# SKA-INAF/caesar-mrcnn

Hardware: AMD Instinct MI355X
Metric: train images/sec (whole node) + detect ms/image, ResNet-101 256x256 (higher is better)
Workload: dtype f32; 1 GPU; resnet101+FPN 256x256 3-class (+bg), nimg_per_gpu=4, train step (fwd+bwd+SGD), 512 train ROIs, 2000 proposals; global_batch=4, parallelism=dp1, weights=random init (Keras defaults)

## Files before the change

caesar-mrcnn_amd/_hip.py:

```python
import ctypes as C
import os
import threading

PKG_DIR = os.path.dirname(os.path.abspath(__file__))
LIB_PATH = os.path.join(PKG_DIR, "libmrcnn_hip.so")


class HipPathError(RuntimeError):
    pass


class ConvDesc(C.Structure):
    _fields_ = [(n, C.c_int32) for n in (
        "N", "H", "W", "Cin", "Cout", "KH", "KW", "stride", "pad_t", "pad_l", "OH", "OW",
        "act", "res_mode", "out_mode", "cmod")] + [
        ("out_n_stride", C.c_int64), ("out_h_stride", C.c_int64), ("out_w_stride", C.c_int64)]


class ConvProblem(C.Structure):
    _fields_ = [("d", ConvDesc)] + [(n, C.c_void_p) for n in ("x", "w", "bias", "scale", "shift", "res", "out", "z_out")]


class WgradProblem(C.Structure):
    _fields_ = [("d", ConvDesc), ("x", C.c_void_p), ("dy", C.c_void_p), ("dw", C.c_void_p), ("accumulate", C.c_int32)]
# ... 125 lines not shown
    "mrcnn_conv2d_wgrad_h16": (C.c_int, [C.POINTER(ConvDesc), C.c_int, _P, _P, _P, _P, C.c_size_t, C.c_int, C.c_float, _P]),
    "mrcnn_mask_out_fwd_h16": (C.c_int, [C.c_int, _P, _P, _P, _P, C.c_int64, C.c_int, C.c_int, _P]),
    "mrcnn_mask_out_bwd_h16": (C.c_int, [C.c_int] + [_P] * 8 + [C.c_int64, C.c_int, C.c_int, C.c_int, C.c_int, C.c_float, _P]),
    "mrcnn_weights_to_h16": (C.c_int, [_P, _P, _P, C.c_int, C.c_int, C.c_int, C.c_int, C.c_int, _P]),
    "mrcnn_weights_to_h16_batched": (C.c_int, [_P, _P, C.c_int, C.c_int, C.c_int, _P]),
    "mrcnn_cast_to_h16": (C.c_int, [_P, _P, C.c_int64, C.c_int, C.c_float, _P]),
    "mrcnn_epilogue_bwd_h16": (C.c_int, [C.c_int] + [_P] * 10 + [C.c_int64, C.c_int, C.c_int, C.c_float, _P]),
    "mrcnn_epilogue_bwd_h16_dy": (C.c_int, [C.c_int] + [_P] * 11 + [C.c_int64, C.c_int, C.c_int, C.c_float, _P]),
    "mrcnn_cast_from_h16": (C.c_int, [_P, _P, C.c_int64, C.c_int, C.c_float, _P]),
    "mrcnn_axpy_from_h16": (C.c_int, [_P, _P, C.c_int64, C.c_int, C.c_float, _P]),
    "mrcnn_rpn_targets_workspace": (C.c_size_t, [C.POINTER(RpnTargetDesc)]),
    "mrcnn_rpn_targets": (C.c_int, [C.POINTER(RpnTargetDesc)] + [_P] * 7 + [C.c_size_t, _P]),
    "mrcnn_detection_workspace": (C.c_size_t, [C.POINTER(DetectionDesc)]),
    "mrcnn_detection_fwd": (C.c_int, [C.POINTER(DetectionDesc)] + [_P] * 6 + [C.c_size_t, _P]),
    "mrcnn_losses_workspace": (C.c_size_t, [C.POINTER(LossDesc)]),
    "mrcnn_losses_fwd_bwd": (C.c_int, [C.POINTER(LossDesc)] + [_P] * 18 + [C.c_size_t, _P]),
    "mrcnn_grad_prepare": (C.c_int, [_P, _P, C.c_float, _P, C.c_int64, _P, _P]),
    "mrcnn_sumsq": (C.c_int, [_P, C.c_int64, _P, _P]),
    "mrcnn_sgd_momentum": (C.c_int, [_P, _P, _P, _P, C.c_float, C.c_float, C.c_float, _P, C.c_int64, _P]),
    "mrcnn_sgd_momentum_guarded": (C.c_int, [_P, _P, _P, _P, C.c_float, C.c_float, C.c_float, _P, C.c_int64, _P, _P]),
    "mrcnn_winograd_buffer_floats": (C.c_size_t, [C.c_int, C.c_int, C.c_int, C.c_int, C.c_int]),
    "mrcnn_winograd_weights": (C.c_int, [_P, _P, C.c_int, C.c_int, C.c_int, _P]),
    "mrcnn_gemm_batched_f32": (C.c_int, [_P, _P, _P, C.c_int, C.c_int, C.c_int, C.c_int, _P]),
    "mrcnn_winograd_gemm": (C.c_int, [_P, _P, _P, C.c_int, C.c_int, C.c_int, C.c_int, _P]),
    "mrcnn_winograd_group_floats": (C.c_size_t, [C.POINTER(WinoGroup), C.c_int, C.c_int]),
    "mrcnn_winograd_input_g": (C.c_int, [_P, _P, C.c_int, C.c_int, C.c_int, C.c_int, C.POINTER(WinoGroup), _P]),
    "mrcnn_winograd_weights_g": (C.c_int, [_P, _P, C.c_int, C.c_int, C.c_int, C.c_int, _P]),
    "mrcnn_winograd_output_g": (C.c_int, [_P, _P, _P, _P, _P, _P, C.c_int, C.c_int, C.c_int, C.c_int, C.c_int, C.POINTER(WinoGroup), _P]),
    "mrcnn_winograd_output_bwd_g": (C.c_int, [_P, _P, _P, _P, _P, _P, _P, _P, _P, _P, C.c_int, C.c_int, C.c_int, C.c_int, C.c_int,
                                             C.POINTER(WinoGroup), _P]),
    "mrcnn_winograd_output_bwd_zmask_g": (C.c_int, [_P] * 10 + [C.c_int, C.c_int, C.c_int, C.c_int, C.POINTER(WinoGroup), _P]),
    "mrcnn_winograd_dy_g": (C.c_int, [_P, _P, C.c_int, C.c_int, C.c_int, C.c_int, C.POINTER(WinoGroup), _P]),
    "mrcnn_winograd_dw_g": (C.c_int, [_P, _P, C.c_int, C.c_int, C.c_int, C.c_int, C.c_int, _P]),
    "mrcnn_deconv2x2_gemm": (C.c_int, [_P, _P, _P, _P, C.c_int, C.c_int, C.c_int, C.c_int, C.c_int, C.c_int, _P]),
    "mrcnn_allreduce_load": (C.c_int, [C.c_char_p]),
    "mrcnn_allreduce_unique_id": (C.c_int, [_P]),
    "mrcnn_allreduce_init": (C.c_int, [C.POINTER(_P), _P, C.c_int, C.c_int]),
    "mrcnn_allreduce_scratch": (C.c_size_t, [C.c_int, C.c_int64, C.c_int]),
    "mrcnn_allreduce_grad": (C.c_int, [_P, _P, C.c_int64, C.c_int64, C.c_int, _P, C.c_size_t, _P]),
    "mrcnn_allreduce_direct_plan": (C.c_int, [C.c_int, C.c_int, C.c_int64, C.c_int64, C.c_int, _P, _P, _P, _P]),
    "mrcnn_allreduce_direct_simulate": (C.c_int, [_P, _P, C.c_size_t, C.c_int, C.c_int64, C.c_int64, _P]),
    "mrcnn_allreduce_destroy": (C.c_int, [_P]),
    "mrcnn_allreduce_last_error": (C.c_char_p, []),
    "mrcnn_tuning_set": (C.c_int, [C.c_char_p, C.c_longlong]),
    "mrcnn_hip_version": (C.c_char_p, []),
}

_lib = None
_proxy = None
_tape = None
_tape_owner = None

_NO_RECORD = ("_workspace", "_tiles_check", "_outline_check", "_draw_check", "_supported", "_status_offset", "_version", "mrcnn_allreduce_", "_scratch", "_floats")


class _LibProxy(object):

    def __init__(self, real):
        self._real = real

    def __getattr__(self, name):
        real = getattr(self._real, name)
        if any(k in name for k in _NO_RECORD):
            f = real
        else:
            def f(*args, _real=real):
# ... 103 lines not shown
```

caesar-mrcnn_amd/csrc/conv_wgrad.hip:

```cpp
#include "common.h"
#include <type_traits>
#include <cstdlib>

struct WgradArgs {
    const float* x; const float* dy; float* out;
    int N, H, W, Cin, Cout, KH, KW, stride, pad_t, pad_l, OH, OW;
    int M, Ktot, fast, splits, chunk, acc;
    FastDiv d_ohw, d_ow;
    const PixelEntry* table;
};

template <int BI, int BN, int WM, int WN>
__global__ __launch_bounds__(WM * WN * 64, 2) void conv_wgrad_kernel(const WgradArgs p) {
    constexpr int NT = WM * WN * 64;
    constexpr int TM = BI / WM / 32, TN = BN / WN / 32;
    constexpr int XST = BI + 4, YST = BN + 4;
    constexpr int XV = 8 * BI / NT, YV = 8 * BN / NT;
    __shared__ __attribute__((aligned(16))) float lds[32 * XST + 32 * YST];
    float* Xs = lds;
    float* Ys = lds + 32 * XST;

    const int tid = threadIdx.x, lane = tid & 63, wave = tid >> 6;
    const int wm = wave / WN, wn = wave % WN;
    const int ntiles = (p.Cout + BN - 1) / BN;
    const int itiles = (p.Ktot + BI - 1) / BI;
    int bid = blockIdx.x;
    const int ntile = bid % ntiles; bid /= ntiles;
    const int itile = bid % itiles;
    const int split = bid / itiles;
    const int i0 = itile * BI, n0 = ntile * BN;
    const int m_begin = split * p.chunk;
    const int m_end = (m_begin + p.chunk < p.M) ? m_begin + p.chunk : p.M;
    const int tap = i0 / p.Cin, ci0 = i0 - tap * p.Cin;
    const int kh = tap / p.KW, kw = tap - kh * p.KW;
    const int ohw = p.OH * p.OW;
// ... 598 lines not shown
    long long blocks = 0, rblocks = 0;
    for (int g = 0; g < n; ++g) {
        const mrcnn_wgrad_problem& q = problems[g];
        const mrcnn_conv_desc* d = &q.d;
        if (!q.x || !q.dy || !q.dw) return MRCNN_ERR_ARG;
        if ((reinterpret_cast<uintptr_t>(q.x) | reinterpret_cast<uintptr_t>(q.dy) | reinterpret_cast<uintptr_t>(q.dw)) & 15)
            return MRCNN_ERR_UNSUPPORTED;
        const long long M = (long long)d->N * d->OH * d->OW;
        WgradArgs& a = mp.a[g];
        a.x = q.x; a.dy = q.dy;
        a.out = pl.splits[g] > 1 ? (float*)((char*)workspace + pl.slab_off[g]) : q.dw;
        a.N = d->N; a.H = d->H; a.W = d->W; a.Cin = d->Cin; a.Cout = d->Cout; a.KH = d->KH; a.KW = d->KW;
        a.stride = d->stride; a.pad_t = d->pad_t; a.pad_l = d->pad_l; a.OH = d->OH; a.OW = d->OW;
        a.M = (int)M; a.Ktot = d->KH * d->KW * d->Cin; a.fast = 1; a.splits = pl.splits[g]; a.chunk = pl.chunk[g];
        a.acc = q.accumulate;
        a.d_ohw = make_fastdiv((unsigned)(d->OH * d->OW)); a.d_ow = make_fastdiv((unsigned)d->OW);
        a.table = nullptr;
        const long long xbytes = (long long)d->N * d->H * d->W * d->Cin * 4;
        const long long shift = ((long long)d->pad_t * d->W + d->pad_l) * d->Cin * 4;
        mp.x_shift[g] = (unsigned)shift; mp.x_records[g] = (unsigned)(xbytes + shift);
        mp.dw[g] = q.dw;
        mp.first[g] = (int)blocks;
        blocks += (long long)(a.Ktot / 128) * (a.Cout / 128) * a.splits;
        mp.rfirst[g] = (int)rblocks;
        if (a.splits > 1) rblocks += cdiv64((long long)a.Ktot * a.Cout / 4, 256);
    }
    for (int g = n; g <= WGRAD_MULTI_MAX; ++g) { mp.first[g] = (int)blocks; mp.rfirst[g] = (int)rblocks; }
    hipStream_t s = (hipStream_t)stream;
    hipLaunchKernelGGL((conv_wgrad_blds_multi_kernel<WGRAD_BP>), dim3((unsigned)blocks), dim3(256), 0, s, mp);
    if (rblocks > 0) hipLaunchKernelGGL(wgrad_reduce_multi_kernel, dim3((unsigned)rblocks), dim3(256), 0, s, mp);
    return mrcnn_launch_status();
}

__global__ void flip_transpose_kernel(const float* __restrict__ w, float* wt, int KH, int KW, int Cin, int Cout) {
    __shared__ float tile[32][33];
    const int tap = blockIdx.z;
    const int kh = tap / KW, kw = tap % KW;
    const int tap_t = (KH - 1 - kh) * KW + (KW - 1 - kw);
    const int ci0 = blockIdx.y * 32, co0 = blockIdx.x * 32;
    const int tx = threadIdx.x & 31, ty = threadIdx.x >> 5;
    for (int r = ty; r < 32; r += 8) {
        int ci = ci0 + r, co = co0 + tx;
        tile[r][tx] = (ci < Cin && co < Cout) ? w[((long long)tap * Cin + ci) * Cout + co] : 0.f;
    }
    __syncthreads();
    for (int r = ty; r < 32; r += 8) {
        int co = co0 + r, ci = ci0 + tx;
        if (co < Cout && ci < Cin) wt[((long long)tap_t * Cout + co) * Cin + ci] = tile[tx][r];
    }
}

extern "C" int mrcnn_weight_flip_transpose(const float* w, float* w_t, int KH, int KW, int Cin, int Cout, void* stream) {
    if (!w || !w_t || KH <= 0 || KW <= 0 || Cin <= 0 || Cout <= 0) return MRCNN_ERR_ARG;
    dim3 grid((Cout + 31) / 32, (Cin + 31) / 32, KH * KW);
    hipLaunchKernelGGL(flip_transpose_kernel, grid, dim3(256), 0, (hipStream_t)stream, w, w_t, KH, KW, Cin, Cout);
    return mrcnn_launch_status();
}

struct FlipEntry { long long off; int KH, KW, Cin, Cout, first_tile, pad; };

__global__ void flip_transpose_batched_kernel(const float* __restrict__ w, float* wt, const FlipEntry* __restrict__ table, int n) {
    __shared__ float tile[32][33];
    int lo = 0, hi = n - 1;
    while (lo < hi) {
        const int mid = (lo + hi + 1) >> 1;
        if (table[mid].first_tile <= (int)blockIdx.x) lo = mid; else hi = mid - 1;
// ... 31 lines not shown
```

caesar-mrcnn_amd/csrc/winograd.hip:

```cpp
#include "common.h"
#include <type_traits>
#include <string.h>

template <int CV> struct WinoVec;
template <> struct WinoVec<4> { typedef f32x4 type; };
template <> struct WinoVec<2> { typedef float type __attribute__((ext_vector_type(2))); };

template <int OT, typename V> __device__ __forceinline__ void wino_bt(const V (&d)[OT + 2], V (&t)[OT + 2]) {
    if constexpr (OT == 2) {
        t[0] = d[0] - d[2];
        t[1] = d[1] + d[2];
        t[2] = d[2] - d[1];
        t[3] = d[1] - d[3];
    } else {
        const V a = d[4] - 4.f * d[2], b = d[3] - 4.f * d[1], c = d[4] - d[2], e = 2.f * (d[3] - d[1]);
        t[0] = 4.f * d[0] - 5.f * d[2] + d[4];
        t[1] = a + b;
        t[2] = a - b;
        t[3] = c + e;
        t[4] = c - e;
        t[5] = 4.f * d[1] - 5.f * d[3] + d[5];
    }
}
template <int OT, typename V> __device__ __forceinline__ void wino_at(const V (&m)[OT + 2], V (&y)[OT]) {
// ... 263 lines not shown
    for (int c = threadIdx.x; c < 3 * CV * L; c += 256) sacc[c] = 0.f;
    __syncthreads();
    const int rsub = threadIdx.x >> lg, lane = threadIdx.x & (L - 1);
    const int c = lane * CV;
    const long long t0 = (long long)blockIdx.x * tiles_per_block;
    long long t1 = t0 + tiles_per_block;
    if (t1 > T) t1 = T;
    vec sc, mu = {}, rs = {}, fsh = {};
#pragma unroll
    for (int e = 0; e < CV; ++e) sc[e] = 1.f;
    if (scale) sc = *(const vec*)(scale + c);
    if (dgamma) { mu = *(const vec*)(mean + c); rs = *(const vec*)(rstd + c); }
    const bool zmask = fwd_shift != nullptr;
    if (zmask) fsh = *(const vec*)(fwd_shift + c);
    vec a_db = {}, a_dg = {}, a_bias = {};
    for (long long t = t0 + rsub; t < t1; t += R)
        wino_output_bwd_tile<OTH, OTW, CV>(Mt, dz_out, below_out, below_z, sc, mu, rs, fsh, zmask, dgamma != nullptr, H, W, C, Tp, act, g, t, c,
                                           a_db, a_dg, a_bias);
#pragma unroll
    for (int k = 0; k < CV; ++k) {
        if (dbeta || dgamma) atomicAdd(&sacc[lane * CV + k], a_db[k]);
        if (dgamma) atomicAdd(&sacc[CV * L + lane * CV + k], a_dg[k]);
        if (dbias) atomicAdd(&sacc[2 * CV * L + lane * CV + k], a_bias[k]);
    }
    __syncthreads();
    for (int j = threadIdx.x; j < CV * L; j += 256) {
        if (dbeta) atomicAdd(&dbeta[j], sacc[j]);
        if (dgamma) atomicAdd(&dgamma[j], sacc[CV * L + j]);
        if (dbias) atomicAdd(&dbias[j], sacc[2 * CV * L + j]);
    }
}

template <int OTH, int OTW, int CV>
__global__ __launch_bounds__(256) void winograd_dy_kernel(const float* __restrict__ dy, float* __restrict__ dM, int N, int H, int W, int C,
                                                          long long T, long long Tp, const WinoGrp g) {
    typedef typename WinoVec<CV>::type vec;
    constexpr int ITH = OTH + 2, ITW = OTW + 2;
    const int cn = C / CV;
    const long long i = (long long)blockIdx.x * 256 + threadIdx.x;
    if (i >= T * cn) return;
    const long long t = i / cn;
    const int c = (int)(i - t * cn) * CV;
    const WinoTile q = wino_tile(t, g.th_n, g.tw_n);
    vec u[ITH][OTW];
#pragma unroll
    for (int b = 0; b < OTW; ++b) {
        vec col[OTH], o[ITH];
#pragma unroll
        for (int a = 0; a < OTH; ++a) {
            const int oh = g.oh0 + OTH * q.th + a, ow = g.ow0 + OTW * q.tw + b;
            vec val = {};
            if (oh < H && ow < W) val = *(const vec*)(dy + (((long long)q.n * H + oh) * W + ow) * C + c);
            col[a] = val;
        }
        wino_a<OTH>(col, o);
#pragma unroll
        for (int r = 0; r < ITH; ++r) u[r][b] = o[r];
    }
#pragma unroll
    for (int r = 0; r < ITH; ++r) {
        vec m[ITW];
        wino_a<OTW>(u[r], m);
#pragma unroll
        for (int k = 0; k < ITW; ++k) *(vec*)(dM + ((long long)(r * ITW + k) * Tp + t) * C + c) = m[k];
    }
}

template <int OTH, int OTW>
__global__ __launch_bounds__(256) void winograd_dw_kernel(const float* __restrict__ dU, float* dW, int Cin, int Cout, int accumulate) {
    constexpr int ITH = OTH + 2, ITW = OTW + 2;
    const long long i = (long long)blockIdx.x * 256 + threadIdx.x;
    const long long n = (long long)Cin * Cout;
    if (i >= n) return;
    float t[3][ITW];
#pragma unroll
    for (int b = 0; b < ITW; ++b) {
        float col[ITH], o[3];
#pragma unroll
        for (int a = 0; a < ITH; ++a) col[a] = dU[(long long)(a * ITW + b) * n + i];
        wino_gt<OTH>(col, o);
#pragma unroll
        for (int a = 0; a < 3; ++a) t[a][b] = o[a];
    }
#pragma unroll
    for (int a = 0; a < 3; ++a) {
        float w[3];
        wino_gt<OTW>(t[a], w);
        float* o = dW + (long long)(a * 3) * n + i;
#pragma unroll
        for (int b = 0; b < 3; ++b) o[b * n] = accumulate ? o[b * n] + w[b] : w[b];
    }
}

typedef __attribute__((address_space(3))) void* wino_lds_ptr;
#define WINO_OOB 0xFFFFFFF0u

struct GemmDeconvEp {
    const float* bias;
    int Cd, H, W, act;
    FastDiv d_hw, d_w;
};

template <int TN, bool DECONV>
__global__ __launch_bounds__(256, 2) void winograd_gemm_kernel(const float* __restrict__ V, const float* __restrict__ U, float* __restrict__ Mt,
                                                               int rows, int K, int N, int total_tiles, unsigned v_records,
                                                               const GemmDeconvEp ep) {
    constexpr int BM = 128, BN = 64 * TN, BK = 16, TM = 2;
    constexpr int AF = BM * BK, BF = BK * BN;
    __shared__ __attribute__((aligned(16))) float lds[2 * (AF + BF)];
    const int tid = threadIdx.x, lane = tid & 63;
    const int wave = __builtin_amdgcn_readfirstlane(tid >> 6);
    const int wm = wave >> 1, wn = wave & 1;
    const int ntiles = N / BN;
    const int nk = K / BK;
    const __amdgpu_buffer_rsrc_t rsrc_a = __builtin_amdgcn_make_buffer_rsrc((void*)V, 0, v_records, 0x00020000);
    const __amdgpu_buffer_rsrc_t rsrc_b = __builtin_amdgcn_make_buffer_rsrc((void*)U, 0, 0x7FFFFFF0u, 0x00020000);

    constexpr int NBP = BF / 256 / 4;
    unsigned a_voff[2], b_voff[4];
    int m0 = 0, n0 = 0;
    auto setup = [&](int tile) {
        const int mtile = tile / ntiles;
        const int ntile = tile - mtile * ntiles;
        m0 = mtile * BM; n0 = ntile * BN;
// ... 204 lines not shown
    if (dgamma && (!below_z || !mean || !rstd)) return MRCNN_ERR_ARG;
    const int cv = wino_grp_cv(g);
    const int cn = C / cv;
    if (cn > 256 || (cn & (cn - 1))) return MRCNN_ERR_UNSUPPORTED;
    int lg = 0;
    while ((1 << lg) < cn) ++lg;
    const long long T = wino_grp_tiles(g, N);
    const long long R = 256 >> lg;
    long long per = (T + 2047) / 2048;
    per = (per + R - 1) / R * R;
    const dim3 grid((unsigned)cdiv64(T, per));
    const WinoGrp k = {g->th_n, g->tw_n, g->oh0, g->ow0};
    WINO_LAUNCH_G(winograd_output_bwd_kernel, g, grid, grid, Mt, dz_below, below_out, below_z, scale, mean, rstd, dgamma, dbeta, dbias, N, H, W,
                  C, T, wino_rows(T), act, per, lg, k, fwd_shift);
    return mrcnn_launch_status();
}

extern "C" int mrcnn_winograd_dy_g(const float* dy, float* dM, int N, int H, int W, int C, const mrcnn_wino_group* g, void* stream) {
    if (!dy || !dM || !wino_grp_ok(g, N, H, W, C)) return MRCNN_ERR_ARG;
    const long long T = wino_grp_tiles(g, N);
    const WinoGrp k = {g->th_n, g->tw_n, g->oh0, g->ow0};
    const dim3 g4((unsigned)cdiv64(T * C / 4, 256)), g2((unsigned)cdiv64(T * C / 2, 256));
    WINO_LAUNCH_G(winograd_dy_kernel, g, g4, g2, dy, dM, N, H, W, C, T, wino_rows(T), k);
    return mrcnn_launch_status();
}

extern "C" int mrcnn_winograd_dw_g(const float* dU, float* dw_hwio, int Cin, int Cout, int accumulate, int oth, int otw, void* stream) {
    if (!dU || !dw_hwio || Cin <= 0 || Cout <= 0 || (oth != 2 && oth != 4) || (otw != 2 && otw != 4)) return MRCNN_ERR_ARG;
    const dim3 grid((unsigned)cdiv64((long long)Cin * Cout, 256));
    WINO_LAUNCH_W(winograd_dw_kernel, oth, otw, grid, dU, dw_hwio, Cin, Cout, accumulate);
    return mrcnn_launch_status();
}

extern "C" size_t mrcnn_winograd_buffer_floats(int N, int H, int W, int C, int tile) {
    if ((tile != 2 && tile != 4) || (tile == 2 && ((H & 1) || (W & 1)))) return 0;
    if (!(N > 0 && H > 0 && W > 0 && C > 0 && !(C & 3))) return 0;
    const mrcnn_wino_group g = {tile, tile, wino_tdim(H, tile), wino_tdim(W, tile), 0, 0};
    return mrcnn_winograd_group_floats(&g, N, C);
}

extern "C" int mrcnn_winograd_weights(const float* w, float* U, int Cin, int Cout, int tile, void* stream) {
    return mrcnn_winograd_weights_g(w, U, Cin, Cout, tile, tile, stream);
}

extern "C" int mrcnn_winograd_gemm(const float* V, const float* U, float* Mt, int nb, int rows, int K, int N, void* stream) {
    if (!V || !U || !Mt || nb <= 0 || rows <= 0 || rows % 128 || K <= 0 || K % 16 || N <= 0 || N % 128) return MRCNN_ERR_ARG;
    const long long M = (long long)nb * rows;
    if (M * K * 4 >= 0x7FFFFFF0LL || (long long)nb * K * N * 4 >= 0x7FFFFFF0LL || M * N >= (1LL << 40)) return MRCNN_ERR_UNSUPPORTED;
    const char* wenv = getenv("MRCNN_WINOGRAD_GEMM_WIDE_MIN");
    const long long wide_min = wenv ? atoll(wenv) : 4096;
    const bool wide = wide_min >= 0 && N % 256 == 0 && (M / 128) * (N / 256) >= wide_min;
    GemmDeconvEp none = {};
    if (wide) {
        const long long tiles = (M / 128) * (N / 256);
        const long long slots = 3LL * mrcnn_num_cus();
        const unsigned grid = (unsigned)(tiles < slots ? tiles : slots);
        hipLaunchKernelGGL((winograd_gemm_kernel<4, false>), dim3(grid), dim3(256), 0, (hipStream_t)stream, V, U, Mt, rows, K, N, (int)tiles,
                           (unsigned)(M * K * 4), none);
        return mrcnn_launch_status();
    }
    const long long tiles = (M / 128) * (N / 128);
    const long long slots = 5LL * mrcnn_num_cus();
    const unsigned grid = (unsigned)(tiles < slots ? tiles : slots);
    hipLaunchKernelGGL((winograd_gemm_kernel<2, false>), dim3(grid), dim3(256), 0, (hipStream_t)stream, V, U, Mt, rows, K, N, (int)tiles,
                       (unsigned)(M * K * 4), none);
    return mrcnn_launch_status();
// ... 22 lines not shown
```

caesar-mrcnn_amd/ops.py:

```python
import ctypes as C
import math
import os

import torch

from . import _hip
from ._hip import (ACT_NONE, ACT_RELU, ACT_SIGMOID, OUT_DECONV2, OUT_NHWC, RES_NONE, RES_SAME, RES_UP2,
                   check, current_stream, ptr)

BN_EPS = 1e-3


def _need_cuda(*ts):
    for t in ts:
        if t is not None and not t.is_cuda:
            raise _hip.HipPathError("hot-path operators need device tensors (got a CPU tensor)")
        if t is not None and not t.is_contiguous():
            raise _hip.HipPathError("hot-path operators need contiguous tensors")


def same_padding(size, k, stride):
    out = -(-size // stride)
    total = max((out - 1) * stride + k - size, 0)
    return out, total // 2
# ... 1258 lines not shown
        out = empty((N, H, W, cout), torch.float32, x.device)
    lib = _hip.lib()

    def finish(g, Mt):
        check(lib.mrcnn_winograd_output_g(ptr(Mt), ptr(out), ptr(z_out), ptr(bias), ptr(scale), ptr(shift), N, H, W, cout, act, C.byref(g),
                                          current_stream()), "mrcnn_winograd_output_g")

    _winograd_run(x, U, finish, keep_v, after_input)
    return out


def conv2d_dgrad_ep_winograd(dz, Ut, below_out, below_z, scale, mean, rstd, dgamma, dbeta, dbias, act, fwd_shift=None):
    _need_cuda(dz, below_out, below_z, scale, mean, rstd, dgamma, dbeta, dbias, fwd_shift)
    N, H, W, _ = dz.shape
    cout = (Ut[0] if isinstance(Ut, (list, tuple)) else Ut).shape[2]
    out = empty((N, H, W, cout), torch.float32, dz.device)
    lib = _hip.lib()
    zmask = act == ACT_RELU and fwd_shift is not None and below_z is not None and scale is not None

    def finish(g, Mt):
        if zmask:
            check(lib.mrcnn_winograd_output_bwd_zmask_g(ptr(Mt), ptr(out), ptr(below_z), ptr(scale), ptr(fwd_shift), ptr(mean), ptr(rstd),
                                                        ptr(dgamma), ptr(dbeta), ptr(dbias), N, H, W, cout, C.byref(g), current_stream()),
                  "mrcnn_winograd_output_bwd_zmask_g")
            return
        check(lib.mrcnn_winograd_output_bwd_g(ptr(Mt), ptr(out), ptr(below_out), ptr(below_z), ptr(scale), ptr(mean), ptr(rstd),
                                              ptr(dgamma), ptr(dbeta), ptr(dbias), N, H, W, cout, act, C.byref(g), current_stream()),
              "mrcnn_winograd_output_bwd_g")

    _winograd_run(dz, Ut, finish)
    return out


def conv2d_wgrad_winograd(V, xshape, dz, dw, accumulate=False, tile=None):
    _need_cuda(V, dz, dw)
    N, H, W, Cin = xshape
    cout = dz.shape[3]
    if tile is None:
        tile = winograd_tile(xshape)
    groups = winograd_groups(H, W, tile)
    lib = _hip.lib()
    nvs = [lib.mrcnn_winograd_group_floats(C.byref(g), N, Cin) for g in groups]
    nms = [lib.mrcnn_winograd_group_floats(C.byref(g), N, cout) for g in groups]
    assert V.numel() == sum(nvs), "V was made with another tiling"
    dM_all = workspace(max(nms) * 4, dz.device, "winograd_dm")
    dU_all = workspace(36 * Cin * cout * 4, dz.device, "winograd_du")
    off = 0
    for gi, g in enumerate(groups):
        nb = _wino_nb(g)
        rows = nms[gi] // (nb * cout)
        T = N * g.th_n * g.tw_n
        dM = dM_all[:nms[gi] * 4].view(torch.float32).view(nb, rows, cout)
        dU = dU_all[:nb * Cin * cout * 4].view(torch.float32).view(nb, Cin, cout)
        check(lib.mrcnn_winograd_dy_g(ptr(dz), ptr(dM), N, H, W, cout, C.byref(g), current_stream()), "mrcnn_winograd_dy_g")
        Vv = V[off:off + nvs[gi]].view(nb, rows, Cin)
        off += nvs[gi]
        items = [(Vv[k, :T].view(T, 1, 1, Cin), dM[k, :T].view(T, 1, 1, cout), (1, 1, Cin, cout), 1, "valid", dU[k].view(1, 1, Cin, cout), False)
                 for k in range(nb)]
        per = 16 if nb == 16 else 12
        for i in range(0, nb, per):
            if not conv2d_wgrad_multi(items[i:i + per]):
                for x_, dy_, wshape, stride, padding, dw_, acc in items[i:i + per]:
                    conv2d_wgrad(x_, dy_, wshape, stride, padding, dw=dw_, accumulate=acc)
        check(lib.mrcnn_winograd_dw_g(ptr(dU), ptr(dw), Cin, cout, 1 if (accumulate or gi > 0) else 0, g.oth, g.otw, current_stream()),
              "mrcnn_winograd_dw_g")
    return dw


def h16_image_table(params, entries, device):
    import numpy as np
    rec = np.zeros(len(entries), dtype=[("off", "<i8"), ("wf", "<u8"), ("wd", "<u8"), ("KH", "<i4"), ("KW", "<i4"), ("Cin", "<i4"),
                                        ("Cout", "<i4"), ("first", "<i4"), ("pad", "<i4")])
    tiles = 0
    for i, (w, wf, wd) in enumerate(entries):
        kh, kw, cin, cout = w.shape
        off = (w.data_ptr() - params.data_ptr()) // 4
        assert 0 <= off and off + w.numel() <= params.numel() and w.is_contiguous()
# ... 136 lines not shown
```

include/mrcnn_hip.h:

```cpp
#ifndef MRCNN_HIP_H
#define MRCNN_HIP_H

#include <stddef.h>
#include <stdint.h>

#ifdef __cplusplus
extern "C" {
#endif

#define MRCNN_OK 0
#define MRCNN_ERR_ARG (-1)
#define MRCNN_ERR_LAUNCH (-2)
#define MRCNN_ERR_WORKSPACE (-3)
#define MRCNN_ERR_UNSUPPORTED (-4)

#define MRCNN_ACT_NONE 0
#define MRCNN_ACT_RELU 1
#define MRCNN_ACT_SIGMOID 2

#define MRCNN_RES_NONE 0
#define MRCNN_RES_SAME 1
#define MRCNN_RES_UP2 2

#define MRCNN_OUT_NHWC 0
// ... 301 lines not shown

int mrcnn_grad_prepare(float* grads, const float* params, float grad_scale, const float* gran_coef,
                       int64_t n, float* sumsq_out, void* stream);
int mrcnn_sumsq(const float* g, int64_t n, float* out_scalar, void* stream);
int mrcnn_sgd_momentum(float* params, float* momentum_buf, const float* grads, const float* sumsq,
                       float clipnorm, float lr, float momentum, const float* gran_coef, int64_t n,
                       void* stream);
int mrcnn_sgd_momentum_guarded(float* params, float* momentum_buf, const float* grads, const float* sumsq,
                               float clipnorm, float lr, float momentum, const float* gran_coef, int64_t n,
                               unsigned* skipped_steps, void* stream);

typedef struct mrcnn_wino_group {
    int oth, otw;
    int th_n, tw_n;
    int oh0, ow0;
} mrcnn_wino_group;
size_t mrcnn_winograd_group_floats(const mrcnn_wino_group* g, int N, int C);
size_t mrcnn_winograd_buffer_floats(int N, int H, int W, int C, int tile);
int mrcnn_winograd_weights(const float* w_hwio, float* U, int Cin, int Cout, int tile, void* stream);
int mrcnn_winograd_weights_g(const float* w_hwio, float* U, int Cin, int Cout, int oth, int otw, void* stream);
int mrcnn_winograd_input_g(const float* x, float* V, int N, int H, int W, int C, const mrcnn_wino_group* g, void* stream);
int mrcnn_gemm_batched_f32(const float* V, const float* U, float* Mt, int nb, int rows, int K, int Cout, void* stream);
int mrcnn_winograd_gemm(const float* V, const float* U, float* Mt, int nb, int rows, int K, int Cout, void* stream);
int mrcnn_winograd_output_g(const float* Mt, float* out, float* z_out, const float* bias, const float* scale, const float* shift,
                            int N, int H, int W, int C, int act, const mrcnn_wino_group* g, void* stream);
int mrcnn_winograd_output_bwd_g(const float* Mt, float* dz_below, const float* below_out, const float* below_z, const float* scale,
                                const float* mean, const float* rstd, float* dgamma, float* dbeta, float* dbias, int N, int H, int W,
                                int C, int act, const mrcnn_wino_group* g, void* stream);
int mrcnn_winograd_output_bwd_zmask_g(const float* Mt, float* dz_below, const float* below_z, const float* scale, const float* shift,
                                      const float* mean, const float* rstd, float* dgamma, float* dbeta, float* dbias, int N, int H,
                                      int W, int C, const mrcnn_wino_group* g, void* stream);
int mrcnn_winograd_dy_g(const float* dy, float* dM, int N, int H, int W, int C, const mrcnn_wino_group* g, void* stream);
int mrcnn_winograd_dw_g(const float* dU, float* dw_hwio, int Cin, int Cout, int accumulate, int oth, int otw, void* stream);

int mrcnn_deconv2x2_gemm(const float* x, const float* w_gemm, const float* bias, float* out, int N, int H, int W, int Cin, int Cd,
                         int act, void* stream);

#define MRCNN_UNIQUE_ID_BYTES 128
#define MRCNN_ALLREDUCE_RCCL 0
#define MRCNN_ALLREDUCE_DIRECT 1
int mrcnn_allreduce_load(const char* librccl_path);
int mrcnn_allreduce_unique_id(void* id_128_bytes);
int mrcnn_allreduce_init(void** comm, const void* id_128_bytes, int rank, int world);
size_t mrcnn_allreduce_scratch(int world, int64_t max_range_floats, int algo);
int mrcnn_allreduce_grad(void* comm, float* grads, int64_t start, int64_t end, int algo, float* scratch,
                         size_t scratch_bytes, void* stream);
int mrcnn_allreduce_direct_plan(int world, int rank, int64_t start, int64_t end, int phase, int64_t* plan, int64_t* own_off,
                                int64_t* own_len, int64_t* slot_stride);
int mrcnn_allreduce_direct_simulate(float* const* grads, float* const* scratch, size_t scratch_bytes, int world, int64_t start,
                                    int64_t end, void* stream);
int mrcnn_allreduce_destroy(void* comm);
const char* mrcnn_allreduce_last_error(void);

int mrcnn_tuning_set(const char* key, long long value);

const char* mrcnn_hip_version(void);

#ifdef __cplusplus
}
#endif
#endif
```

Measured before the change: 111.9 images/s.

## Batch Winograd weight-gradient across tile groups into single split-K launches

Winograd weight-gradient previously ran per tile group: one dy transform, batched GEMMs and one dw inverse transform each. Now a single kernel transforms dy for all groups, one multi-group split-K GEMM kernel writes partial slabs, and a single kernel reduces the slabs and applies the inverse transform. The goal is fewer launches and better GPU occupancy on small spatial sizes, at the cost of a larger workspace and extra slab memory traffic. It falls back to the old per-group path when the plan is unsupported.

```diff
diff --git a/caesar-mrcnn_amd/_hip.py b/caesar-mrcnn_amd/_hip.py
--- a/caesar-mrcnn_amd/_hip.py
+++ b/caesar-mrcnn_amd/_hip.py
@@ -181,6 +181,12 @@
     "mrcnn_winograd_output_bwd_zmask_g": (C.c_int, [_P] * 10 + [C.c_int, C.c_int, C.c_int, C.c_int, C.POINTER(WinoGroup), _P]),
     "mrcnn_winograd_dy_g": (C.c_int, [_P, _P, C.c_int, C.c_int, C.c_int, C.c_int, C.POINTER(WinoGroup), _P]),
     "mrcnn_winograd_dw_g": (C.c_int, [_P, _P, C.c_int, C.c_int, C.c_int, C.c_int, C.c_int, _P]),
+    "mrcnn_winograd_wgrad_plan": (C.c_int, [C.POINTER(WinoGroup), C.c_int, C.c_int, C.c_int, C.c_int, C.c_int, C.POINTER(C.c_int),
+                                           C.POINTER(C.c_int), C.POINTER(C.c_size_t)]),
+    "mrcnn_winograd_wgrad_gemms_workspace": (C.c_size_t, [C.POINTER(WinoGroup), C.c_int, C.c_int, C.c_int, C.c_int, C.c_int]),
+    "mrcnn_winograd_dy_all": (C.c_int, [_P, _P, C.c_int, C.c_int, C.c_int, C.c_int, C.POINTER(WinoGroup), C.c_int, _P]),
+    "mrcnn_winograd_wgrad_gemms": (C.c_int, [C.POINTER(WinoGroup), C.c_int, _P, _P, C.c_int, C.c_int, C.c_int, C.c_int, _P, C.c_size_t, _P]),
+    "mrcnn_winograd_dw_slabs": (C.c_int, [C.POINTER(WinoGroup), C.c_int, _P, C.c_int, C.c_int, C.c_int, C.c_int, _P, C.c_int, _P]),
     "mrcnn_deconv2x2_gemm": (C.c_int, [_P, _P, _P, _P, C.c_int, C.c_int, C.c_int, C.c_int, C.c_int, C.c_int, _P]),
     "mrcnn_allreduce_load": (C.c_int, [C.c_char_p]),
     "mrcnn_allreduce_unique_id": (C.c_int, [_P]),
diff --git a/caesar-mrcnn_amd/csrc/conv_wgrad.hip b/caesar-mrcnn_amd/csrc/conv_wgrad.hip
--- a/caesar-mrcnn_amd/csrc/conv_wgrad.hip
+++ b/caesar-mrcnn_amd/csrc/conv_wgrad.hip
@@ -1,6 +1,7 @@
 #include "common.h"
 #include <type_traits>
 #include <cstdlib>
+#include <string.h>
 
 struct WgradArgs {
     const float* x; const float* dy; float* out;
@@ -665,6 +666,113 @@
     return mrcnn_launch_status();
 }
 
+struct WinoWgradGroup {
+    WgradArgs a;
+    long long x_step, dy_step, out_step;
+    unsigned x_records;
+    int first, per;
+};
+struct WinoWgradArgs { WinoWgradGroup g[MRCNN_WINO_MAX_GROUPS]; int n; };
+
+template <int BP>
+__global__ __launch_bounds__(256, 2) void winograd_wgrad_gemms_kernel(const WinoWgradArgs mp) {
+    int g = 0;
+    while (g + 1 < mp.n && (int)blockIdx.x >= mp.g[g + 1].first) ++g;
+    const WinoWgradGroup& q = mp.g[g];
+    const int b = (int)blockIdx.x - q.first;
+    const int k = b / q.per;
+    WgradArgs a = q.a;
+    a.x += k * q.x_step; a.dy += k * q.dy_step; a.out += k * q.out_step;
+    conv_wgrad_blds_body<BP, false>(a, 0u, q.x_records, b - k * q.per);
+}
+
+#define WINO_WGRAD_TARGET 2048
+
+extern "C" int mrcnn_winograd_wgrad_plan(const mrcnn_wino_group* groups, int n_groups, int N, int Cin, int Cout, int chunk_in,
+                                         int* chunk_out, int* splits_out, size_t* slab_bytes_out) {
+    if (!groups || n_groups < 1 || n_groups > MRCNN_WINO_MAX_GROUPS || N <= 0 || Cin <= 0 || Cout <= 0 || chunk_in < 0) return MRCNN_ERR_ARG;
+    if (Cin % 128 || Cout % 128) return MRCNN_ERR_UNSUPPORTED;
+    long long T[MRCNN_WINO_MAX_GROUPS], nb[MRCNN_WINO_MAX_GROUPS], Tmax = 0;
+    for (int g = 0; g < n_groups; ++g) {
+        const mrcnn_wino_group& q = groups[g];
+        if ((q.oth != 2 && q.oth != 4) || (q.otw != 2 && q.otw != 4) || q.th_n <= 0 || q.tw_n <= 0) return MRCNN_ERR_ARG;
+        T[g] = (long long)N * q.th_n * q.tw_n;
+        nb[g] = (q.oth + 2) * (q.otw + 2);
+        const long long big = Cin > Cout ? Cin : Cout;
+        if ((T[g] + 16) * big * 4 >= 0x7FFFFFF0LL) return MRCNN_ERR_UNSUPPORTED;
+        if (T[g] > Tmax) Tmax = T[g];
+    }
+    const long long tiles = (long long)(Cin / 128) * (Cout / 128);
+    auto groups_of = [&](long long chunk) {
+        long long wg = 0;
+        for (int g = 0; g < n_groups; ++g) wg += nb[g] * tiles * ((T[g] + chunk - 1) / chunk);
+        return wg;
+    };
+    long long chunk;
+    if (chunk_in > 0) chunk = ((long long)chunk_in + 31) / 32 * 32;
+    else {
+        chunk = (Tmax + 31) / 32 * 32;
+        for (long long s = 2; s <= 64; ++s) {
+            const long long c = ((Tmax + s - 1) / s + 31) / 32 * 32;
+            if (c < 256 || groups_of(c) > WINO_WGRAD_TARGET) break;
+            chunk = c;
+        }
+    }
+    size_t bytes = 0;
+    for (int g = 0; g < n_groups; ++g) {
+        const long long s = (T[g] + chunk - 1) / chunk;
+        if (splits_out) splits_out[g] = (int)s;
+        bytes += (size_t)(nb[g] * s) * Cin * Cout * sizeof(float);
+    }
+    if (groups_of(chunk) >= (1LL << 31)) return MRCNN_ERR_UNSUPPORTED;
+    if (chunk_out) *chunk_out = (int)chunk;
+    if (slab_bytes_out) *slab_bytes_out = bytes;
+    return MRCNN_OK;
+}
+
+extern "C" size_t mrcnn_winograd_wgrad_gemms_workspace(const mrcnn_wino_group* groups, int n_groups, int N, int Cin, int Cout, int chunk) {
+    size_t bytes = 0;
+    if (mrcnn_winograd_wgrad_plan(groups, n_groups, N, Cin, Cout, chunk, nullptr, nullptr, &bytes) != MRCNN_OK) return 0;
+    return bytes;
+}
+
+extern "C" int mrcnn_winograd_wgrad_gemms(const mrcnn_wino_group* groups, int n_groups, const float* V, const float* dM, int N, int Cin,
+                                          int Cout, int chunk, float* workspace, size_t workspace_bytes, void* stream) {
+    int splits[MRCNN_WINO_MAX_GROUPS], ch = 0;
+    size_t bytes = 0;
+    const int rc = mrcnn_winograd_wgrad_plan(groups, n_groups, N, Cin, Cout, chunk, &ch, splits, &bytes);
+    if (rc != MRCNN_OK) return rc;
+    if (mrcnn_force_flat_glds()) return MRCNN_ERR_UNSUPPORTED;
+    if (!V || !dM) return MRCNN_ERR_ARG;
+    if ((reinterpret_cast<uintptr_t>(V) | reinterpret_cast<uintptr_t>(dM)) & 15) return MRCNN_ERR_UNSUPPORTED;
+    if (!workspace || workspace_bytes < bytes || (reinterpret_cast<uintptr_t>(workspace) & 15)) return MRCNN_ERR_WORKSPACE;
+    WinoWgradArgs mp;
+    memset(&mp, 0, sizeof(mp));
+    mp.n = n_groups;
+    const long long tiles = (long long)(Cin / 128) * (Cout / 128);
+    long long blocks = 0;
+    const float* v = V; const float* dm = dM; float* slab = workspace;
+    for (int g = 0; g < n_groups; ++g) {
+        const mrcnn_wino_group& q = groups[g];
+        const long long T = (long long)N * q.th_n * q.tw_n, rows = (T + 127) / 128 * 128, nb = (q.oth + 2) * (q.otw + 2);
+        WinoWgradGroup& w = mp.g[g];
+        WgradArgs& a = w.a;
+        a.x = v; a.dy = dm; a.out = slab;
+        a.N = (int)T; a.H = 1; a.W = 1; a.Cin = Cin; a.Cout = Cout; a.KH = 1; a.KW = 1;
+        a.stride = 1; a.pad_t = 0; a.pad_l = 0; a.OH = 1; a.OW = 1;
+        a.M = (int)T; a.Ktot = Cin; a.fast = 1; a.splits = splits[g]; a.chunk = ch; a.acc = 0;
+        a.d_ohw = make_fastdiv(1u); a.d_ow = make_fastdiv(1u);
+        a.table = nullptr;
+        w.x_step = rows * Cin; w.dy_step = rows * Cout; w.out_step = (long long)splits[g] * Cin * Cout;
+        w.x_records = (unsigned)(T * Cin * 4);
+        w.first = (int)blocks; w.per = (int)(tiles * splits[g]);
+        blocks += nb * w.per;
+        v += nb * w.x_step; dm += nb * w.dy_step; slab += nb * w.out_step;
+    }
+    hipLaunchKernelGGL((winograd_wgrad_gemms_kernel<WGRAD_BP>), dim3((unsigned)blocks), dim3(256), 0, (hipStream_t)stream, mp);
+    return mrcnn_launch_status();
+}
+
 __global__ void flip_transpose_kernel(const float* __restrict__ w, float* wt, int KH, int KW, int Cin, int Cout) {
     __shared__ float tile[32][33];
     const int tap = blockIdx.z;
diff --git a/caesar-mrcnn_amd/csrc/winograd.hip b/caesar-mrcnn_amd/csrc/winograd.hip
--- a/caesar-mrcnn_amd/csrc/winograd.hip
+++ b/caesar-mrcnn_amd/csrc/winograd.hip
@@ -319,12 +319,11 @@
 }
 
 template <int OTH, int OTW, int CV>
-__global__ __launch_bounds__(256) void winograd_dy_kernel(const float* __restrict__ dy, float* __restrict__ dM, int N, int H, int W, int C,
-                                                          long long T, long long Tp, const WinoGrp g) {
+__device__ __forceinline__ void winograd_dy_body(const float* __restrict__ dy, float* __restrict__ dM, int N, int H, int W, int C,
+                                                 long long T, long long Tp, const WinoGrp g, const long long i) {
     typedef typename WinoVec<CV>::type vec;
     constexpr int ITH = OTH + 2, ITW = OTW + 2;
     const int cn = C / CV;
-    const long long i = (long long)blockIdx.x * 256 + threadIdx.x;
     if (i >= T * cn) return;
     const long long t = i / cn;
     const int c = (int)(i - t * cn) * CV;
@@ -351,6 +350,31 @@
 #pragma unroll
         for (int k = 0; k < ITW; ++k) *(vec*)(dM + ((long long)(r * ITW + k) * Tp + t) * C + c) = m[k];
     }
+}
+
+template <int OTH, int OTW, int CV>
+__global__ __launch_bounds__(256) void winograd_dy_kernel(const float* __restrict__ dy, float* __restrict__ dM, int N, int H, int W, int C,
+                                                          long long T, long long Tp, const WinoGrp g) {
+    winograd_dy_body<OTH, OTW, CV>(dy, dM, N, H, W, C, T, Tp, g, (long long)blockIdx.x * 256 + threadIdx.x);
+}
+
+struct WinoDyAllArgs {
+    WinoGrp g[MRCNN_WINO_MAX_GROUPS];
+    long long T[MRCNN_WINO_MAX_GROUPS], Tp[MRCNN_WINO_MAX_GROUPS], off[MRCNN_WINO_MAX_GROUPS];
+    int oth[MRCNN_WINO_MAX_GROUPS], otw[MRCNN_WINO_MAX_GROUPS], first[MRCNN_WINO_MAX_GROUPS + 1];
+    int n;
+};
+
+__global__ __launch_bounds__(256) void winograd_dy_all_kernel(const float* __restrict__ dy, float* __restrict__ dM, int N, int H, int W, int C,
+                                                              const WinoDyAllArgs p) {
+    int k = 0;
+    while (k + 1 < p.n && (int)blockIdx.x >= p.first[k + 1]) ++k;
+    const long long i = (long long)((int)blockIdx.x - p.first[k]) * 256 + threadIdx.x;
+    float* out = dM + p.off[k];
+    if (p.oth[k] == 2 && p.otw[k] == 2) winograd_dy_body<2, 2, 4>(dy, out, N, H, W, C, p.T[k], p.Tp[k], p.g[k], i);
+    else if (p.oth[k] == 4 && p.otw[k] == 4) winograd_dy_body<4, 4, 2>(dy, out, N, H, W, C, p.T[k], p.Tp[k], p.g[k], i);
+    else if (p.oth[k] == 4) winograd_dy_body<4, 2, 2>(dy, out, N, H, W, C, p.T[k], p.Tp[k], p.g[k], i);
+    else winograd_dy_body<2, 4, 2>(dy, out, N, H, W, C, p.T[k], p.Tp[k], p.g[k], i);
 }
 
 template <int OTH, int OTW>
@@ -377,6 +401,77 @@
 #pragma unroll
         for (int b = 0; b < 3; ++b) o[b * n] = accumulate ? o[b * n] + w[b] : w[b];
     }
+}
+
+template <int OTH, int OTW>
+__device__ __forceinline__ void winograd_dw_slabs_group(const float* __restrict__ slab, const int splits, const long long n, const long long i,
+                                                        float (&w)[3][3]) {
+    constexpr int ITH = OTH + 2, ITW = OTW + 2;
+    float t[3][ITW];
+#pragma unroll
+    for (int b = 0; b < ITW; ++b) {
+        float col[ITH], o[3];
+#pragma unroll
+        for (int a = 0; a < ITH; ++a) col[a] = 0.f;
+        for (int k0 = 0; k0 < splits; k0 += 8) {
+            float v[ITH][8];
+#pragma unroll
+            for (int a = 0; a < ITH; ++a)
+#pragma unroll
+                for (int j = 0; j < 8; ++j) {
+                    int k = k0 + j;
+                    if (k > splits - 1) k = splits - 1;
+                    v[a][j] = slab[((long long)(a * ITW + b) * splits + k) * n + i];
+                }
+#pragma unroll
+            for (int a = 0; a < ITH; ++a)
+#pragma unroll
+                for (int j = 0; j < 8; ++j)
+                    if (k0 + j < splits) col[a] += v[a][j];
+        }
+        wino_gt<OTH>(col, o);
+#pragma unroll
+        for (int a = 0; a < 3; ++a) t[a][b] = o[a];
+    }
+#pragma unroll
+    for (int a = 0; a < 3; ++a) {
+        float r[3];
+        wino_gt<OTW>(t[a], r);
+#pragma unroll
+        for (int b = 0; b < 3; ++b) w[a][b] += r[b];
+    }
+}
+
+struct WinoDwSlabsArgs {
+    long long off[MRCNN_WINO_MAX_GROUPS];
+    int splits[MRCNN_WINO_MAX_GROUPS], oth[MRCNN_WINO_MAX_GROUPS], otw[MRCNN_WINO_MAX_GROUPS];
+    int n;
+};
+
+__global__ __launch_bounds__(256) void winograd_dw_slabs_kernel(const float* __restrict__ slabs, float* dW, int Cin, int Cout, int accumulate,
+                                                                const WinoDwSlabsArgs p) {
+    const long long i = (long long)blockIdx.x * 256 + threadIdx.x;
+    const long long n = (long long)Cin * Cout;
+    if (i >= n) return;
+    float w[3][3];
+#pragma unroll
+    for (int a = 0; a < 3; ++a)
+#pragma unroll
+        for (int b = 0; b < 3; ++b) w[a][b] = 0.f;
+    for (int g = 0; g < p.n; ++g) {
+        const float* s = slabs + p.off[g];
+        if (p.oth[g] == 2 && p.otw[g] == 2) winograd_dw_slabs_group<2, 2>(s, p.splits[g], n, i, w);
+        else if (p.oth[g] == 4 && p.otw[g] == 4) winograd_dw_slabs_group<4, 4>(s, p.splits[g], n, i, w);
+        else if (p.oth[g] == 4) winograd_dw_slabs_group<4, 2>(s, p.splits[g], n, i, w);
+        else winograd_dw_slabs_group<2, 4>(s, p.splits[g], n, i, w);
+    }
+#pragma unroll
+    for (int a = 0; a < 3; ++a)
+#pragma unroll
+        for (int b = 0; b < 3; ++b) {
+            float* o = dW + (long long)(a * 3 + b) * n + i;
+            *o = accumulate ? *o + w[a][b] : w[a][b];
+        }
 }
 
 typedef __attribute__((address_space(3))) void* wino_lds_ptr;
@@ -647,6 +742,48 @@
     return mrcnn_launch_status();
 }
 
+extern "C" int mrcnn_winograd_dy_all(const float* dy, float* dM, int N, int H, int W, int C, const mrcnn_wino_group* groups, int n_groups,
+                                     void* stream) {
+    if (!dy || !dM || !groups || n_groups < 1 || n_groups > MRCNN_WINO_MAX_GROUPS) return MRCNN_ERR_ARG;
+    WinoDyAllArgs p;
+    memset(&p, 0, sizeof(p));
+    p.n = n_groups;
+    long long blocks = 0, off = 0;
+    for (int k = 0; k < n_groups; ++k) {
+        const mrcnn_wino_group* g = groups + k;
+        if (!wino_grp_ok(g, N, H, W, C)) return MRCNN_ERR_ARG;
+        const long long T = wino_grp_tiles(g, N);
+        p.g[k] = WinoGrp{g->th_n, g->tw_n, g->oh0, g->ow0};
+        p.T[k] = T; p.Tp[k] = wino_rows(T); p.off[k] = off;
+        p.oth[k] = g->oth; p.otw[k] = g->otw;
+        p.first[k] = (int)blocks;
+        blocks += cdiv64(T * C / wino_grp_cv(g), 256);
+        off += (long long)wino_grp_nb(g) * wino_rows(T) * C;
+    }
+    if (blocks >= (1LL << 31)) return MRCNN_ERR_UNSUPPORTED;
+    for (int k = n_groups; k <= MRCNN_WINO_MAX_GROUPS; ++k) p.first[k] = (int)blocks;
+    hipLaunchKernelGGL(winograd_dy_all_kernel, dim3((unsigned)blocks), dim3(256), 0, (hipStream_t)stream, dy, dM, N, H, W, C, p);
+    return mrcnn_launch_status();
+}
+
+extern "C" int mrcnn_winograd_dw_slabs(const mrcnn_wino_group* groups, int n_groups, const float* slabs, int N, int Cin, int Cout, int chunk,
+                                       float* dw_hwio, int accumulate, void* stream) {
+    if (!slabs || !dw_hwio) return MRCNN_ERR_ARG;
+    WinoDwSlabsArgs p;
+    memset(&p, 0, sizeof(p));
+    const int rc = mrcnn_winograd_wgrad_plan(groups, n_groups, N, Cin, Cout, chunk, nullptr, p.splits, nullptr);
+    if (rc != MRCNN_OK) return rc;
+    p.n = n_groups;
+    long long off = 0;
+    for (int k = 0; k < n_groups; ++k) {
+        p.off[k] = off; p.oth[k] = groups[k].oth; p.otw[k] = groups[k].otw;
+        off += (long long)wino_grp_nb(groups + k) * p.splits[k] * Cin * Cout;
+    }
+    const dim3 grid((unsigned)cdiv64((long long)Cin * Cout, 256));
+    hipLaunchKernelGGL(winograd_dw_slabs_kernel, grid, dim3(256), 0, (hipStream_t)stream, slabs, dw_hwio, Cin, Cout, accumulate, p);
+    return mrcnn_launch_status();
+}
+
 extern "C" size_t mrcnn_winograd_buffer_floats(int N, int H, int W, int C, int tile) {
     if ((tile != 2 && tile != 4) || (tile == 2 && ((H & 1) || (W & 1)))) return 0;
     if (!(N > 0 && H > 0 && W > 0 && C > 0 && !(C & 3))) return 0;
diff --git a/caesar-mrcnn_amd/ops.py b/caesar-mrcnn_amd/ops.py
--- a/caesar-mrcnn_amd/ops.py
+++ b/caesar-mrcnn_amd/ops.py
@@ -1314,6 +1314,24 @@
     return out
 
 
+_WINO_WGRAD_CHUNK = int(os.environ.get("MRCNN_WINOGRAD_WGRAD_CHUNK", "0"))
+
+
+def winograd_wgrad_plan(xshape, cout, tile=None, chunk=None):
+    N, H, W, Cin = xshape
+    if tile is None:
+        tile = winograd_tile(xshape)
+    groups = winograd_groups(H, W, tile)
+    arr = (_hip.WinoGroup * len(groups))(*groups)
+    ch, splits, nbytes = C.c_int(0), (C.c_int * len(groups))(), C.c_size_t(0)
+    rc = _hip.lib().mrcnn_winograd_wgrad_plan(arr, len(groups), N, Cin, cout, _WINO_WGRAD_CHUNK if chunk is None else chunk, C.byref(ch),
+                                              splits, C.byref(nbytes))
+    if rc == ERR_UNSUPPORTED:
+        return None
+    check(rc, "mrcnn_winograd_wgrad_plan")
+    return ch.value, list(splits), nbytes.value, [N * g.th_n * g.tw_n for g in groups]
+
+
 def conv2d_wgrad_winograd(V, xshape, dz, dw, accumulate=False, tile=None):
     _need_cuda(V, dz, dw)
     N, H, W, Cin = xshape
@@ -1325,6 +1343,28 @@
     nvs = [lib.mrcnn_winograd_group_floats(C.byref(g), N, Cin) for g in groups]
     nms = [lib.mrcnn_winograd_group_floats(C.byref(g), N, cout) for g in groups]
     assert V.numel() == sum(nvs), "V was made with another tiling"
+    arr = (_hip.WinoGroup * len(groups))(*groups)
+    chunk = _WINO_WGRAD_CHUNK
+    nbytes = lib.mrcnn_winograd_wgrad_gemms_workspace(arr, len(groups), N, Cin, cout, chunk)
+    if nbytes == 0:
+        return _conv2d_wgrad_winograd_groups(V, xshape, dz, dw, accumulate, groups, nvs, nms)
+    dM = workspace(sum(nms) * 4, dz.device, "winograd_dm")
+    slabs = workspace(nbytes, dz.device, "winograd_slabs")
+    st = current_stream()
+    check(lib.mrcnn_winograd_dy_all(ptr(dz), ptr(dM), N, H, W, cout, arr, len(groups), st), "mrcnn_winograd_dy_all")
+    rc = lib.mrcnn_winograd_wgrad_gemms(arr, len(groups), ptr(V), ptr(dM), N, Cin, cout, chunk, ptr(slabs), slabs.numel(), st)
+    if rc == ERR_UNSUPPORTED:
+        return _conv2d_wgrad_winograd_groups(V, xshape, dz, dw, accumulate, groups, nvs, nms)
+    check(rc, "mrcnn_winograd_wgrad_gemms")
+    check(lib.mrcnn_winograd_dw_slabs(arr, len(groups), ptr(slabs), N, Cin, cout, chunk, ptr(dw), 1 if accumulate else 0, st),
+          "mrcnn_winograd_dw_slabs")
+    return dw
+
+
+def _conv2d_wgrad_winograd_groups(V, xshape, dz, dw, accumulate, groups, nvs, nms):
+    N, H, W, Cin = xshape
+    cout = dz.shape[3]
+    lib = _hip.lib()
     dM_all = workspace(max(nms) * 4, dz.device, "winograd_dm")
     dU_all = workspace(36 * Cin * cout * 4, dz.device, "winograd_du")
     off = 0
diff --git a/include/mrcnn_hip.h b/include/mrcnn_hip.h
--- a/include/mrcnn_hip.h
+++ b/include/mrcnn_hip.h
@@ -357,6 +357,16 @@
                                       int W, int C, const mrcnn_wino_group* g, void* stream);
 int mrcnn_winograd_dy_g(const float* dy, float* dM, int N, int H, int W, int C, const mrcnn_wino_group* g, void* stream);
 int mrcnn_winograd_dw_g(const float* dU, float* dw_hwio, int Cin, int Cout, int accumulate, int oth, int otw, void* stream);
+#define MRCNN_WINO_MAX_GROUPS 4
+int mrcnn_winograd_wgrad_plan(const mrcnn_wino_group* groups, int n_groups, int N, int Cin, int Cout, int chunk, int* chunk_out,
+                              int* splits_out, size_t* slab_bytes_out);
+size_t mrcnn_winograd_wgrad_gemms_workspace(const mrcnn_wino_group* groups, int n_groups, int N, int Cin, int Cout, int chunk);
+int mrcnn_winograd_dy_all(const float* dy, float* dM, int N, int H, int W, int C, const mrcnn_wino_group* groups, int n_groups,
+                          void* stream);
+int mrcnn_winograd_wgrad_gemms(const mrcnn_wino_group* groups, int n_groups, const float* V, const float* dM, int N, int Cin, int Cout,
+                               int chunk, float* workspace, size_t workspace_bytes, void* stream);
+int mrcnn_winograd_dw_slabs(const mrcnn_wino_group* groups, int n_groups, const float* slabs, int N, int Cin, int Cout, int chunk,
+                            float* dw_hwio, int accumulate, void* stream);
 
 int mrcnn_deconv2x2_gemm(const float* x, const float* w_gemm, const float* bias, float* out, int N, int H, int W, int Cin, int Cd,
                          int act, void* stream);
```

New measurement: 111.6 images/s. Within noise of the previous version (-0.3%).
